# haidog-yaqub/EzAudio

Hardware: AMD Instinct MI355X
Metric: denoising steps/sec (EzAudio-XL, 10 s latent, CFG on) (higher is better)
Workload: dtype bf16

## Files before the change

ezaudio_amd/csrc/attn.hip:

```cpp
#include "common.h"

namespace {

typedef __attribute__((ext_vector_type(4))) short s16x4;

__device__ __forceinline__ float pair_max(float x) {
    const auto r = __builtin_amdgcn_permlane32_swap(__float_as_uint(x), __float_as_uint(x), false, false);
    return fmaxf(__uint_as_float(r[0]), __uint_as_float(r[1]));
}
__device__ __forceinline__ float pair_sum(float x) {
    const auto r = __builtin_amdgcn_permlane32_swap(__float_as_uint(x), __float_as_uint(x), false, false);
    return __uint_as_float(r[0]) + __uint_as_float(r[1]);
}

template <int DH>
struct HeadGeom;
template <>
struct HeadGeom<64> { static constexpr int DQK = 64, DV = 64; };
template <>
struct HeadGeom<72> { static constexpr int DQK = 80, DV = 96; };

template <int DH, int NKH, bool ZQ = false, int QT = 64>
__global__ __launch_bounds__(128 * NKH) void k_attn(AttnArgs a) {
    static_assert(QT == 64 || (QT == 32 && NKH == 4), "32-query tiles: the 8-wave fused-projection form only");
    constexpr int NQS = QT / 32;
    constexpr int NT = 128 * NKH;
    constexpr int TK = 32 * NKH;
    constexpr int DQK = HeadGeom<DH>::DQK;
    constexpr int DV = HeadGeom<DH>::DV;
    constexpr int NKS = DQK / 16;
    constexpr int NDT = DV / 32;
    constexpr int KSTR = DQK * 2 + 16;
    constexpr int VSTR = 192;
    static_assert(DV * 2 <= VSTR, "V row");
    constexpr int KBYTES = TK * KSTR, VBYTES = TK * VSTR;
    constexpr int BUF = KBYTES + VBYTES;
    constexpr int KCH = TK * DQK * 2 / 16;
    constexpr int VCPR = DV / 8;
    constexpr int VCH = TK * VCPR;
    constexpr int KPT = (KCH + NT - 1) / NT, VPT = (VCH + NT - 1) / NT;
    static_assert(KPT <= 3 && VPT <= 3, "staging registers");
    constexpr int DN = DV >= 96 ? 96 : 64;
    constexpr int DW = DQK;
    constexpr int DS = DQK;
    constexpr int NRS = QT == 64 ? 3 : 4;
    constexpr int PSTAGE = (QT + DN) * 128, PRING = 2 * NRS * PSTAGE;
    constexpr int PRED = 4 * 64 * DS * 4, PQS = QT * DQK * 2;
    constexpr int SMEM = NKH == 4 ? (2 * BUF > PRED + PQS ? (2 * BUF > PRING ? 2 * BUF : PRING) : (PRED + PQS > PRING ? PRED + PQS : PRING)) : 2 * BUF;
    constexpr int ZX = ZQ ? QT * 8 + 2 * DQK * 4 : 0;
    __shared__ __attribute__((aligned(16))) char smem[SMEM + ZX];

    int Lq_ = a.Lq;
    asm("" : "+s"(Lq_) : "s"(a.q), "s"(a.k), "s"(a.v), "s"(a.kmask), "s"(a.out), "s"(a.ldo), "s"(a.B), "s"(a.H), "s"(a.Lk), "s"(a.Lqp), "s"(a.Lkp), "s"(a.xu), "s"(a.ldu),
        "s"(a.xw), "s"(a.ldw), "s"(a.xw_rows), "s"(a.xK), "s"(a.xcd_map), "s"(a.nq), "s"(a.ppx), "s"(a.mnq), "s"(a.mH), "s"(a.q_raw), "s"(a.ts), "s"(a.xk2), "s"(a.zstat_in),
        "s"(a.zs_stride), "s"(a.zparts), "s"(a.klen));
    const int tid = threadIdx.x;
    const int lane = tid & 63;
    const int wave = tid >> 6;
    const int qs = QT == 64 ? (wave & 1) : 0, kh = QT == 64 ? (wave >> 1) : (wave & 3);
    const bool active = QT == 64 || __builtin_amdgcn_readfirstlane(wave) < 4;
    const int r32 = lane & 31, hi = lane >> 5;
    int qt, h, b;
    if (a.xcd_map) {
        const int xcd = blockIdx.x & 7, sl = blockIdx.x >> 3;
        const int sq = ez_div(sl, a.mnq);
        const int pair = xcd * a.ppx + sq;
        qt = sl - sq * a.nq;
        if (pair >= a.B * a.H) return;
        b = ez_div(pair, a.mH); h = pair - b * a.H;
    } else {
        qt = blockIdx.x; h = blockIdx.y; b = blockIdx.z;
    }
    const int q0 = qt * QT + qs * 32;
    const long bh = (long)b * a.H + h;
    int Lk = a.Lk;
    if constexpr (!ZQ) {
        if (a.klen) {
            Lk = __builtin_amdgcn_readfirstlane(a.klen[b]);
            if (qt * QT >= Lk) {
                for (int i = tid; i < QT * (DH / 4); i += NT) {
                    const int r = i / (DH / 4), g = i - r * (DH / 4);
                    if (qt * QT + r < a.Lq)
                        *reinterpret_cast<uint2*>(a.out + ((long)b * a.Lq + qt * QT + r) * a.ldo + h * DH + 4 * g) = make_uint2(0u, 0u);
                }
                return;
            }
        }
    }
    unsigned long long* ts = (a.ts && tid < 64) ? a.ts + 8 * (long)blockIdx.x : nullptr;
    if (ts && lane == 0) { ts[0] = __builtin_readcyclecounter(); ts[6] = ez_stamp_start(); }

    const bf16_t* Q = a.q + (bh * a.Lqp + q0 + r32) * DQK + 8 * hi;
    const char* Kg = reinterpret_cast<const char*>(a.k + bh * a.Lkp * DQK);
    const bf16_t* Vg = a.v + bh * DV * (long)a.Lkp;
    const uint8_t* km = a.kmask ? a.kmask + (long)b * a.Lk : nullptr;

    bf16x8 qf[NKS];
    if (NKH == 4 && a.xu) {
        if constexpr (NKH == 4) {
            constexpr int FN = DN / 32;
            constexpr int NPART = QT == 64 ? 4 : 8;
            const int rowb = b * a.Lq;
            float2* zrow_l = reinterpret_cast<float2*>(smem + SMEM);
            float* zgc_l = reinterpret_cast<float*>(smem + SMEM + QT * 8);
            ZStatRegs zst;
            float4 zgc_reg = make_float4(0.f, 0.f, 0.f, 0.f);
            const int wave_u = __builtin_amdgcn_readfirstlane(wave);
            const char* gA = reinterpret_cast<const char*>(a.xu);
            const char* gW = reinterpret_cast<const char*>(a.xw);
            const int nt = a.xK / 64;
            auto z_request = [&]() {
                if constexpr (ZQ) {
                    if (tid < 4 * QT) {
                        int qr = qt * QT + (tid >> 2);
                        qr = qr < a.Lq ? qr : a.Lq - 1;
                        z_row_stats_load(a.zstat_in + (rowb + qr), a.zs_stride, a.zparts, tid & 3, zst);
                    }
                    if (tid < 2 * (DH / 4)) {
                        const int which = tid >= DH / 4, t4 = tid - which * (DH / 4);
                        zgc_reg = *reinterpret_cast<const float4*>((which ? a.zC : a.zG) + h * DH + 4 * t4);
                    }
                }
            };
            f32x16 acc[FN];
#pragma unroll
            for (int j = 0; j < FN; ++j)
#pragma unroll
                for (int r = 0; r < 16; ++r) acc[j][r] = 0.f;
            if constexpr (QT == 32) {
                constexpr int NCH = (32 + DW) * 8, NW1 = (NCH - NT) / 64;
                static_assert(NCH > NT && NCH <= 2 * NT && (NCH - NT) % 64 == 0, "two passes, whole waves");
                uint32_t off0, off1;
                {
                    const int row = tid >> 3, c = tid & 7;
                    if (row < 32) {
                        int grow = rowb + qt * 32 + row;
                        grow = grow < rowb + a.Lq - 1 ? grow : rowb + a.Lq - 1;
                        off0 = (uint32_t)(grow * a.ldu + ((c ^ ((row >> 1) & 7)) << 3)) * 2u;
                    } else {
                        const int r2 = row - 32;
                        int gr = h * DH + r2;
                        gr = gr < a.xw_rows - 1 ? gr : a.xw_rows - 1;
                        off0 = (uint32_t)(gr * a.ldw + ((c ^ ((r2 >> 1) & 7)) << 3)) * 2u;
                    }
                    const int r2 = (tid >> 3) + 32;
                    int gr = h * DH + r2;
                    gr = gr < a.xw_rows - 1 ? gr : a.xw_rows - 1;
                    off1 = (uint32_t)(gr * a.ldw + ((c ^ ((r2 >> 1) & 7)) << 3)) * 2u;
                }
                const char* g0 = wave_u < 4 ? gA : gW;
                const bool two = wave_u < NW1;
                auto stage2 = [&](int sidx) {
                    char* dst = smem + (sidx % NRS) * 2 * PSTAGE + wave_u * 1024;
#pragma unroll
                    for (int sub = 0; sub < 2; ++sub) {
                        const long ko = (long)(2 * sidx + sub) * 128;
                        __builtin_amdgcn_global_load_lds((const __attribute__((address_space(1))) void*)(g0 + ko + off0),
                                                         (__attribute__((address_space(3))) void*)(dst + sub * PSTAGE), 16, 0, 0);
                        if (two)
                            __builtin_amdgcn_global_load_lds((const __attribute__((address_space(1))) void*)(gW + ko + off1),
                                                             (__attribute__((address_space(3))) void*)(dst + sub * PSTAGE + NT * 16), 16, 0, 0);
                    }
                };
                const int ns = nt >> 1;
                stage2(0);
                z_request();
                if (ns > 1) stage2(1);
                if (ns > 2) stage2(2);
                const int sub = wave_u >> 2, kq = wave_u & 3;
                const uint32_t fo = r32 * 128 + (((2 * kq + hi) ^ ((r32 >> 1) & 7)) << 4);
                for (int sidx = 0; sidx < ns; ++sidx) {
                    const int younger = ns - 1 - sidx < NRS - 2 ? ns - 1 - sidx : NRS - 2;
                    if (two) {
                        if (younger >= 2) asm volatile("s_waitcnt vmcnt(8)" ::: "memory");
                        else if (younger == 1) asm volatile("s_waitcnt vmcnt(4)" ::: "memory");
                        else asm volatile("s_waitcnt vmcnt(0)" ::: "memory");
                    } else {
                        if (younger >= 2) asm volatile("s_waitcnt vmcnt(4)" ::: "memory");
                        else if (younger == 1) asm volatile("s_waitcnt vmcnt(2)" ::: "memory");
                        else asm volatile("s_waitcnt vmcnt(0)" ::: "memory");
                    }
                    __builtin_amdgcn_s_barrier();
                    if (sidx + NRS - 1 < ns) stage2(sidx + NRS - 1);
                    const char* cT = smem + (sidx % NRS) * 2 * PSTAGE + sub * PSTAGE;
                    const bf16x8 af = *reinterpret_cast<const bf16x8*>(cT + fo);
#pragma unroll
                    for (int j = 0; j < FN; ++j) {
                        const bf16x8 bfr = *reinterpret_cast<const bf16x8*>(cT + 32 * 128 + fo + j * 4096);
                        acc[j] = __builtin_amdgcn_mfma_f32_32x32x16_bf16(bfr, af, acc[j], 0, 0, 0);
                    }
#pragma unroll
                    for (int j = 0; j < FN; ++j) asm volatile("" : "+a"(acc[j]));
                }
            } else {
            const int mh = wave & 1, kq = wave >> 1;
            uint32_t aoff[1], boff[(DW * 8 + NT - 1) / NT];
            stage_offsets<64, NT>(aoff, a.ldu, rowb + qt * 64, rowb + a.Lq - 1, tid);
            stage_offsets<DW, NT>(boff, a.ldw, h * DH, a.xw_rows - 1, tid);
            auto stage = [&](int t) {
                char* dst = smem + (t % 3) * PSTAGE + wave_u * 1024;
                stage_tile<64, NT>(gA + (long)t * 128, aoff, dst, tid);
                stage_tile<DW, NT>(gW + (long)t * 128, boff, dst + 64 * 128, tid);
            };
            const bool two = (DW * 8 > NT) && (wave_u * 64 + NT < DW * 8);
            stage(0);
            if (nt > 1) stage(1);
            z_request();
            const uint32_t fo = r32 * 128 + (((2 * kq + hi) ^ ((r32 >> 1) & 7)) << 4);
            if (a.xk2 && (nt & 1) == 0) {
                const int ns = nt >> 1;
                auto stage2 = [&](int sidx) {
                    char* dst = smem + (sidx % 3) * 2 * PSTAGE + wave_u * 1024;
#pragma unroll
                    for (int sub = 0; sub < 2; ++sub) {
                        stage_tile<64, NT>(gA + (long)(2 * sidx + sub) * 128, aoff, dst + sub * PSTAGE, tid);
                        stage_tile<DW, NT>(gW + (long)(2 * sidx + sub) * 128, boff, dst + sub * PSTAGE + 64 * 128, tid);
                    }
                };
                if (ns > 1) stage2(1);
                for (int sidx = 0; sidx < ns; ++sidx) {
                    if (sidx + 1 < ns) {
                        if (two) asm volatile("s_waitcnt vmcnt(6)" ::: "memory"); else asm volatile("s_waitcnt vmcnt(4)" ::: "memory");
                    } else {
                        asm volatile("s_waitcnt vmcnt(0)" ::: "memory");
                    }
                    __builtin_amdgcn_s_barrier();
                    if (sidx + 2 < ns) stage2(sidx + 2);
#pragma unroll
                    for (int sub = 0; sub < 2; ++sub) {
                        const char* cT = smem + (sidx % 3) * 2 * PSTAGE + sub * PSTAGE;
                        const bf16x8 af = *reinterpret_cast<const bf16x8*>(cT + fo + mh * 4096);
#pragma unroll
                        for (int j = 0; j < FN; ++j) {
                            const bf16x8 bfr = *reinterpret_cast<const bf16x8*>(cT + 64 * 128 + fo + j * 4096);
                            acc[j] = __builtin_amdgcn_mfma_f32_32x32x16_bf16(bfr, af, acc[j], 0, 0, 0);
                        }
                    }
#pragma unroll
                    for (int j = 0; j < FN; ++j) asm volatile("" : "+a"(acc[j]));
                }
            } else
            for (int t = 0; t < nt; ++t) {
                if (t + 1 < nt) {
                    if (two) asm volatile("s_waitcnt vmcnt(3)" ::: "memory"); else asm volatile("s_waitcnt vmcnt(2)" ::: "memory");
                } else {
                    asm volatile("s_waitcnt vmcnt(0)" ::: "memory");
                }
                __builtin_amdgcn_s_barrier();
                if (t + 2 < nt) stage(t + 2);
                const char* cT = smem + (t % 3) * PSTAGE;
                const bf16x8 af = *reinterpret_cast<const bf16x8*>(cT + fo + mh * 4096);
#pragma unroll
                for (int j = 0; j < FN; ++j) {
                    const bf16x8 bfr = *reinterpret_cast<const bf16x8*>(cT + 64 * 128 + fo + j * 4096);
                    acc[j] = __builtin_amdgcn_mfma_f32_32x32x16_bf16(bfr, af, acc[j], 0, 0, 0);
                }
#pragma unroll
                for (int j = 0; j < FN; ++j) asm volatile("" : "+a"(acc[j]));
            }
            }
#pragma unroll
            for (int j = 0; j < FN; ++j) asm volatile("s_nop 7\n\ts_nop 7\n\ts_nop 3" : "+a"(acc[j]));
            if constexpr (ZQ) {
                if (tid < 4 * QT) {
                    const float2 mr = z_row_stats_finish(zst, a.zparts, tid & 3, a.zD, a.zeps);
                    if ((tid & 3) == 0) zrow_l[tid >> 2] = mr;
                }
                if (tid < 2 * (DH / 4)) {
                    const int which = tid >= DH / 4, t4 = tid - which * (DH / 4);
                    *reinterpret_cast<float4*>(zgc_l + which * DQK + 4 * t4) = zgc_reg;
                }
            }
            __syncthreads();
            float* red = reinterpret_cast<float*>(smem);
            {
                const int pw = QT == 64 ? (wave >> 1) : wave, prow = QT == 64 ? 32 * (wave & 1) + r32 : r32;
#pragma unroll
                for (int j = 0; j < FN; ++j)
#pragma unroll
                    for (int g = 0; g < 4; ++g) {
                        const int col = 32 * j + 8 * g + 4 * hi;
                        if (col < DS)
                            *reinterpret_cast<float4*>(red + ((pw * QT + prow) * DS + col)) =
                                make_float4(acc[j][4 * g], acc[j][4 * g + 1], acc[j][4 * g + 2], acc[j][4 * g + 3]);
                    }
            }
            __syncthreads();
            if (QT == 64 || tid < 8 * QT) {
                constexpr int CP = DH / 8;
                bf16_t* qs_l = reinterpret_cast<bf16_t*>(smem + PRED);
                const int row = tid >> 3, part = tid & 7;
                float v[CP];
                float s1 = 0.f;
                const float2 zmr = ZQ ? zrow_l[row] : make_float2(0.f, 1.f);
                const float zmu = zmr.x, zr = zmr.y;
#pragma unroll
                for (int e = 0; e < CP; ++e) {
                    const int col = part * CP + e;
                    if constexpr (QT == 64) {
                        v[e] = red[(0 * 64 + row) * DS + col] + red[(1 * 64 + row) * DS + col] + red[(2 * 64 + row) * DS + col] +
                               red[(3 * 64 + row) * DS + col];
                    } else {
                        float t = red[row * DS + col];
#pragma unroll
                        for (int w = 1; w < NPART; ++w) t += red[(w * QT + row) * DS + col];
                        v[e] = t;
                    }
                    if constexpr (ZQ) v[e] = fmaf(zr, v[e], fmaf(-zr * zmu, zgc_l[col], zgc_l[DQK + col]));
                    s1 += v[e];
                }
                s1 = oct_sum(s1);
                const float mean = s1 * (1.f / DH);
                float s2 = 0.f;
#pragma unroll
                for (int e = 0; e < CP; ++e) { const float d = v[e] - mean; s2 += d * d; }
                s2 = oct_sum(s2);
                const float rstd = rsqrtf(s2 * (1.f / DH) + 1e-5f);
#pragma unroll
                for (int e = 0; e < CP; ++e) {
                    const int col = part * CP + e;
                    qs_l[row * DQK + col] = f2bf((v[e] - mean) * rstd * a.qn_w[col] + a.qn_b[col]);
                }
                if (DQK > DH && part == 0)
                    for (int col = DH; col < DQK; ++col) qs_l[row * DQK + col] = 0;
            }
            __syncthreads();
            {
                const bf16_t* qs_l = reinterpret_cast<const bf16_t*>(smem + PRED);
#pragma unroll
                for (int ks = 0; ks < NKS; ++ks) qf[ks] = *reinterpret_cast<const bf16x8*>(qs_l + (32 * qs + r32) * DQK + 16 * ks + 8 * hi);
            }
            __syncthreads();
        }
    } else if (a.q_raw) {
        int qr = q0 + r32;
        if (qr >= a.Lq) qr = a.Lq - 1;
        const float* src = a.q_raw + ((long)b * a.Lq + qr) * a.ld_qraw + h * DH + 8 * hi;
        float v[NKS][8];
        float s = 0.f;
#pragma unroll
        for (int ks = 0; ks < NKS; ++ks) {
            const bool ok = 16 * ks + 8 * hi < DH;
            const float4 lo = ok ? *reinterpret_cast<const float4*>(src + 16 * ks) : make_float4(0.f, 0.f, 0.f, 0.f);
            const float4 hh = ok ? *reinterpret_cast<const float4*>(src + 16 * ks + 4) : make_float4(0.f, 0.f, 0.f, 0.f);
            v[ks][0] = lo.x; v[ks][1] = lo.y; v[ks][2] = lo.z; v[ks][3] = lo.w;
            v[ks][4] = hh.x; v[ks][5] = hh.y; v[ks][6] = hh.z; v[ks][7] = hh.w;
#pragma unroll
            for (int e = 0; e < 8; ++e) s += v[ks][e];
        }
        s += __shfl_xor(s, 32, 64);
        const float mean = s * (1.f / DH);
        float q2 = 0.f;
#pragma unroll
        for (int ks = 0; ks < NKS; ++ks)
            if (16 * ks + 8 * hi < DH) {
#pragma unroll
                for (int e = 0; e < 8; ++e) { const float d = v[ks][e] - mean; q2 += d * d; }
            }
        q2 += __shfl_xor(q2, 32, 64);
        const float rstd = rsqrtf(q2 * (1.f / DH) + 1e-5f);
#pragma unroll
        for (int ks = 0; ks < NKS; ++ks) {
            const int d0 = 16 * ks + 8 * hi;
            const bool ok = d0 < DH;
            const int dw = ok ? d0 : 0;
            union { bf16x8 v; uint32_t u[4]; } pk;
#pragma unroll
            for (int e = 0; e < 4; ++e) {
                const float y0 = ok ? (v[ks][2 * e] - mean) * rstd * a.qn_w[dw + 2 * e] + a.qn_b[dw + 2 * e] : 0.f;
                const float y1 = ok ? (v[ks][2 * e + 1] - mean) * rstd * a.qn_w[dw + 2 * e + 1] + a.qn_b[dw + 2 * e + 1] : 0.f;
                pk.u[e] = pack_bf2(y0, y1);
            }
            qf[ks] = pk.v;
        }
    } else {
#pragma unroll
        for (int ks = 0; ks < NKS; ++ks) qf[ks] = *reinterpret_cast<const bf16x8*>(Q + 16 * ks);
    }

    uint4 k0 = {}, k1 = {}, k2 = {}, v0 = {}, v1 = {}, v2 = {};
    uint32_t koff[3], voff[3];
#pragma unroll
    for (int i = 0; i < 3; ++i) {
        int ck = tid + NT * i, cv = tid + NT * i;
        ck = ck < KCH ? ck : KCH - 1;
        cv = cv < VCH ? cv : VCH - 1;
        koff[i] = (uint32_t)ck * 16u;
        voff[i] = (uint32_t)cv * 16u;
    }
    const __amdgpu_buffer_rsrc_t krs = __builtin_amdgcn_make_buffer_rsrc(const_cast<char*>(Kg), 0, a.Lkp * DQK * 2, 0x00020000);
    const __amdgpu_buffer_rsrc_t vrs = __builtin_amdgcn_make_buffer_rsrc(const_cast<bf16_t*>(Vg), 0, DV * a.Lkp * 2, 0x00020000);
    auto kchunk = [&](int i, int key0) -> uint4 {
        return __builtin_bit_cast(uint4, __builtin_amdgcn_raw_buffer_load_b128(krs, (int)koff[i], key0 * DQK * 2, 0));
    };
    auto vchunk = [&](int i, int key0) -> uint4 {
        return __builtin_bit_cast(uint4, __builtin_amdgcn_raw_buffer_load_b128(vrs, (int)voff[i], key0 * DV * 2, 0));
    };
    auto kstore = [&](int i, char* kb, const uint4& val) {
        const int c = tid + NT * i;
        if (c < KCH) *reinterpret_cast<uint4*>(kb + (c / (DQK / 8)) * KSTR + (c % (DQK / 8)) * 16) = val;
    };
    auto vstore = [&](int i, char* vb, const uint4& val) {
        const int c = tid + NT * i;
        if (c < VCH) *reinterpret_cast<uint4*>(vb + (c / VCPR) * VSTR + (c % VCPR) * 16) = val;
    };
#define LOAD_TILE(t)                                   \
    do {                                               \
        const int key0_ = (t) * TK;                    \
        k0 = kchunk(0, key0_);                         \
        k1 = kchunk(1, key0_);                         \
        if constexpr (KPT > 2) k2 = kchunk(2, key0_);  \
        v0 = vchunk(0, key0_);                         \
        v1 = vchunk(1, key0_);                         \
        if constexpr (VPT > 2) v2 = vchunk(2, key0_);  \
    } while (0)
#define WRITE_TILE(buf)                                \
    do {                                               \
        char* kb_ = smem + (buf) * BUF;                \
        char* vb_ = kb_ + KBYTES;                      \
        kstore(0, kb_, k0);                            \
        kstore(1, kb_, k1);                            \
        if constexpr (KPT > 2) kstore(2, kb_, k2);     \
        vstore(0, vb_, v0);                            \
        vstore(1, vb_, v1);                            \
        if constexpr (VPT > 2) vstore(2, vb_, v2);     \
    } while (0)

    f32x16 o[NDT];
#pragma unroll
    for (int t = 0; t < NDT; ++t)
#pragma unroll
        for (int r = 0; r < 16; ++r) o[t][r] = 0.f;
    float m = -1e30f, lsum = 0.f;
    constexpr float RESCALE_THR = 4.0f;
    const float c = 1.4426950408889634f * rsqrtf((float)DH);

    if (NKH == 4 && __builtin_amdgcn_readfirstlane(threadIdx.x) >= 256) __builtin_amdgcn_s_setprio(1);
    const int ntiles = (Lk + TK - 1) / TK;
    LOAD_TILE(0);
    WRITE_TILE(0);
    __syncthreads();
    if (ts && lane == 0) ts[1] = __builtin_readcyclecounter();
    for (int t = 0; t < ntiles; ++t) {
        if (t + 1 < ntiles) LOAD_TILE(t + 1);
        const char* kb = smem + (t & 1) * BUF;
        const char* vb = kb + KBYTES;
        const char* vtr = vb + (32 * kh + 4 * hi + ((lane & 15) >> 2)) * VSTR + ((lane & 16) + 4 * (lane & 3)) * 2;
        const int key0 = t * TK + kh * 32;
        if (active && key0 < Lk) {
            const int kidx = key0 + r32;
            bool kv = kidx < Lk;
            if (km) kv = kv && (km[kidx < Lk ? kidx : 0] != 0);
            const uint32_t ball = (uint32_t)__ballot(kv);
            const uint32_t tmask = ball >> (4 * hi);
            const bool full = ball == 0xffffffffu;
            f32x16 s;
            {
                const bf16x8 kf0 = *reinterpret_cast<const bf16x8*>(kb + (kh * 32 + r32) * KSTR + hi * 16);
                asm("s_nop 1\n\tv_mfma_f32_32x32x16_bf16 %0, %1, %2, 0" : "=&v"(s) : "v"(kf0), "v"(qf[0]));
            }
#pragma unroll
            for (int ks = 1; ks < NKS; ++ks) {
                const bf16x8 kf = *reinterpret_cast<const bf16x8*>(kb + (kh * 32 + r32) * KSTR + (2 * ks + hi) * 16);
                if (ks + 1 < NKS) asm("s_nop 1\n\tv_mfma_f32_32x32x16_bf16 %0, %1, %2, %0" : "+v"(s) : "v"(kf), "v"(qf[ks]));
                else asm("s_nop 1\n\tv_mfma_f32_32x32x16_bf16 %0, %1, %2, %0\n\ts_nop 7\n\ts_nop 7\n\ts_nop 3" : "+v"(s) : "v"(kf), "v"(qf[ks]));
            }
            float tmax = -1e30f;
            if (full) {
#pragma unroll
                for (int r = 0; r < 16; ++r) tmax = fmaxf(tmax, s[r]);
                tmax *= c;
            } else {
#pragma unroll
                for (int r = 0; r < 16; ++r) {
                    const bool v = (tmask >> ((r & 3) + 8 * (r >> 2))) & 1u;
                    s[r] = v ? s[r] * c : -1e30f;
                    tmax = fmaxf(tmax, s[r]);
                }
            }
            tmax = pair_max(tmax);
            if (!__all(tmax <= m + RESCALE_THR)) {
                const float mnew = fmaxf(m, tmax);
                const float alpha = __builtin_amdgcn_exp2f(m - mnew);
                m = mnew;
                lsum *= alpha;
#pragma unroll
                for (int tt = 0; tt < NDT; ++tt)
#pragma unroll
                    for (int r = 0; r < 16; ++r) o[tt][r] *= alpha;
            }
            float psum = 0.f;
            float p[16];
            if (full) {
                const f32x2 c2 = {c, c}, nm2 = {-m, -m};
                f32x2 ps2 = {0.f, 0.f};
#pragma unroll
                for (int r = 0; r < 16; r += 2) {
                    f32x2 x = {s[r], s[r + 1]};
                    x = __builtin_elementwise_fma(x, c2, nm2);
                    p[r] = __builtin_amdgcn_exp2f(x[0]);
                    p[r + 1] = __builtin_amdgcn_exp2f(x[1]);
                    const f32x2 pp = {p[r], p[r + 1]};
                    ps2 += pp;
                }
                psum = ps2[0] + ps2[1];
// ... 78 lines not shown
                }
                if (a.wt) st8_wt(orow + 8 * G, v); else *reinterpret_cast<uint2*>(orow + 8 * G) = v;
            }
        }
    }
    if (ts && lane == 0) { asm volatile("s_waitcnt vmcnt(0)" ::: "memory"); ts[3] = __builtin_readcyclecounter(); ts[7] = __builtin_amdgcn_s_memrealtime(); }
}

#undef LOAD_TILE
#undef WRITE_TILE

}

int launch_attention(const AttnArgs& a0, hipStream_t st) {
    AttnArgs a = a0;
    if (a.b0 > 0) {
        const int DQK = a.dh == 64 ? 64 : 80, DV = a.dh == 64 ? 64 : 96;
        const long b0 = a.b0;
        if (a.q) a.q += b0 * a.H * a.Lqp * DQK;
        if (a.k) a.k += b0 * a.H * a.Lkp * DQK;
        if (a.v) a.v += b0 * a.H * DV * (long)a.Lkp;
        if (a.kmask) a.kmask += b0 * a.Lk;
        if (a.out) a.out += b0 * a.Lq * a.ldo;
        if (a.q_raw) a.q_raw += b0 * a.Lq * a.ld_qraw;
        if (a.xu) a.xu += b0 * a.Lq * a.ldu;
        if (a.zstat_in) a.zstat_in += b0 * a.Lq;
        if (a.klen) a.klen += b0;
        a.b0 = 0;
    }
    const long nwg64 = (long)((a.Lq + 63) / 64) * a.H * a.B;
    int nkh = a.nkh;
    if (nkh != 2 && nkh != 4) nkh = nwg64 <= 512 ? 4 : 2;
    if (a.Lkp % 128) nkh = 2;
    if (a.xu && nkh != 4) return 1;
    if (a.dh != 64 && a.dh != 72) return 1;
    if (a.klen && (a.xu || a.q_raw || a.Lq != a.Lk)) return 1;
    const bool zq = a.xu && a.zstat_in;
    if (zq && !(a.zG && a.zC && a.zparts > 0 && a.zparts <= Z_MAXP && a.zs_stride > 0 && a.zw > 0)) return 1;
    const bool q32 = zq && nkh == 4 && (a.xK / 64) % 2 == 0 && a.xcd_map && (a.qtile == 32 || (a.qtile == 0 && nwg64 <= 128));
    const int QT = q32 ? 32 : 64;
    a.nq = (a.Lq + QT - 1) / QT;
    a.ppx = (a.B * a.H + 7) / 8;
    a.mnq = ez_magic(a.nq); a.mH = ez_magic(a.H);
    dim3 grid(a.nq, a.H, a.B);
    if (a.xcd_map) grid = dim3(8 * a.ppx * a.nq, 1, 1);
    if (a.ts && (long)grid.x * grid.y * grid.z > a.ts_cap) a.ts = nullptr;
    if (q32) {
        if (a.dh == 64) hipLaunchKernelGGL((k_attn<64, 4, true, 32>), grid, dim3(512), 0, st, a);
        else hipLaunchKernelGGL((k_attn<72, 4, true, 32>), grid, dim3(512), 0, st, a);
        return 0;
    }
    if (a.dh == 64) {
        if (nkh == 4 && zq) hipLaunchKernelGGL((k_attn<64, 4, true>), grid, dim3(512), 0, st, a);
        else if (nkh == 4) hipLaunchKernelGGL((k_attn<64, 4>), grid, dim3(512), 0, st, a);
        else hipLaunchKernelGGL((k_attn<64, 2>), grid, dim3(256), 0, st, a);
    } else {
        if (nkh == 4 && zq) hipLaunchKernelGGL((k_attn<72, 4, true>), grid, dim3(512), 0, st, a);
        else if (nkh == 4) hipLaunchKernelGGL((k_attn<72, 4>), grid, dim3(512), 0, st, a);
        else hipLaunchKernelGGL((k_attn<72, 2>), grid, dim3(256), 0, st, a);
    }
    return 0;
}
```

Measured before the change: 269.4.

## Overlap first K/V tile and mask loads with fused Q projection prologue

```diff
diff --git a/ezaudio_amd/csrc/attn.hip b/ezaudio_amd/csrc/attn.hip
--- a/ezaudio_amd/csrc/attn.hip
+++ b/ezaudio_amd/csrc/attn.hip
@@ -20,8 +20,9 @@
 template <>
 struct HeadGeom<72> { static constexpr int DQK = 80, DV = 96; };
 
-template <int DH, int NKH, bool ZQ = false, int QT = 64>
+template <int DH, int NKH, bool ZQ = false, int QT = 64, bool XU = ZQ>
 __global__ __launch_bounds__(128 * NKH) void k_attn(AttnArgs a) {
+    static_assert((!ZQ || XU) && (!XU || NKH == 4), "the fused projection: 8-wave form; the LayerNorm algebra: fused projection only");
     static_assert(QT == 64 || (QT == 32 && NKH == 4), "32-query tiles: the 8-wave fused-projection form only");
     constexpr int NQS = QT / 32;
     constexpr int NT = 128 * NKH;
@@ -47,13 +48,17 @@
     constexpr int PSTAGE = (QT + DN) * 128, PRING = 2 * NRS * PSTAGE;
     constexpr int PRED = 4 * 64 * DS * 4, PQS = QT * DQK * 2;
     constexpr int SMEM = NKH == 4 ? (2 * BUF > PRED + PQS ? (2 * BUF > PRING ? 2 * BUF : PRING) : (PRED + PQS > PRING ? PRED + PQS : PRING)) : 2 * BUF;
-    constexpr int ZX = ZQ ? QT * 8 + 2 * DQK * 4 : 0;
+    constexpr int ZXZ = ZQ ? QT * 8 + 2 * DQK * 4 : 0;
+    constexpr int ZX = ZXZ + (XU ? 2 * DQK * 4 : 0);
     __shared__ __attribute__((aligned(16))) char smem[SMEM + ZX];
 
     int Lq_ = a.Lq;
     asm("" : "+s"(Lq_) : "s"(a.q), "s"(a.k), "s"(a.v), "s"(a.kmask), "s"(a.out), "s"(a.ldo), "s"(a.B), "s"(a.H), "s"(a.Lk), "s"(a.Lqp), "s"(a.Lkp), "s"(a.xu), "s"(a.ldu),
         "s"(a.xw), "s"(a.ldw), "s"(a.xw_rows), "s"(a.xK), "s"(a.xcd_map), "s"(a.nq), "s"(a.ppx), "s"(a.mnq), "s"(a.mH), "s"(a.q_raw), "s"(a.ts), "s"(a.xk2), "s"(a.zstat_in),
         "s"(a.zs_stride), "s"(a.zparts), "s"(a.klen));
+    const float* qn_w_ = a.qn_w;
+    const float* qn_b_ = a.qn_b;
+    asm("" : "+s"(qn_w_), "+s"(qn_b_));
     const int tid = threadIdx.x;
     const int lane = tid & 63;
     const int wave = tid >> 6;
@@ -94,289 +99,6 @@
     const char* Kg = reinterpret_cast<const char*>(a.k + bh * a.Lkp * DQK);
     const bf16_t* Vg = a.v + bh * DV * (long)a.Lkp;
     const uint8_t* km = a.kmask ? a.kmask + (long)b * a.Lk : nullptr;
-
-    bf16x8 qf[NKS];
-    if (NKH == 4 && a.xu) {
-        if constexpr (NKH == 4) {
-            constexpr int FN = DN / 32;
-            constexpr int NPART = QT == 64 ? 4 : 8;
-            const int rowb = b * a.Lq;
-            float2* zrow_l = reinterpret_cast<float2*>(smem + SMEM);
-            float* zgc_l = reinterpret_cast<float*>(smem + SMEM + QT * 8);
-            ZStatRegs zst;
-            float4 zgc_reg = make_float4(0.f, 0.f, 0.f, 0.f);
-            const int wave_u = __builtin_amdgcn_readfirstlane(wave);
-            const char* gA = reinterpret_cast<const char*>(a.xu);
-            const char* gW = reinterpret_cast<const char*>(a.xw);
-            const int nt = a.xK / 64;
-            auto z_request = [&]() {
-                if constexpr (ZQ) {
-                    if (tid < 4 * QT) {
-                        int qr = qt * QT + (tid >> 2);
-                        qr = qr < a.Lq ? qr : a.Lq - 1;
-                        z_row_stats_load(a.zstat_in + (rowb + qr), a.zs_stride, a.zparts, tid & 3, zst);
-                    }
-                    if (tid < 2 * (DH / 4)) {
-                        const int which = tid >= DH / 4, t4 = tid - which * (DH / 4);
-                        zgc_reg = *reinterpret_cast<const float4*>((which ? a.zC : a.zG) + h * DH + 4 * t4);
-                    }
-                }
-            };
-            f32x16 acc[FN];
-#pragma unroll
-            for (int j = 0; j < FN; ++j)
-#pragma unroll
-                for (int r = 0; r < 16; ++r) acc[j][r] = 0.f;
-            if constexpr (QT == 32) {
-                constexpr int NCH = (32 + DW) * 8, NW1 = (NCH - NT) / 64;
-                static_assert(NCH > NT && NCH <= 2 * NT && (NCH - NT) % 64 == 0, "two passes, whole waves");
-                uint32_t off0, off1;
-                {
-                    const int row = tid >> 3, c = tid & 7;
-                    if (row < 32) {
-                        int grow = rowb + qt * 32 + row;
-                        grow = grow < rowb + a.Lq - 1 ? grow : rowb + a.Lq - 1;
-                        off0 = (uint32_t)(grow * a.ldu + ((c ^ ((row >> 1) & 7)) << 3)) * 2u;
-                    } else {
-                        const int r2 = row - 32;
-                        int gr = h * DH + r2;
-                        gr = gr < a.xw_rows - 1 ? gr : a.xw_rows - 1;
-                        off0 = (uint32_t)(gr * a.ldw + ((c ^ ((r2 >> 1) & 7)) << 3)) * 2u;
-                    }
-                    const int r2 = (tid >> 3) + 32;
-                    int gr = h * DH + r2;
-                    gr = gr < a.xw_rows - 1 ? gr : a.xw_rows - 1;
-                    off1 = (uint32_t)(gr * a.ldw + ((c ^ ((r2 >> 1) & 7)) << 3)) * 2u;
-                }
-                const char* g0 = wave_u < 4 ? gA : gW;
-                const bool two = wave_u < NW1;
-                auto stage2 = [&](int sidx) {
-                    char* dst = smem + (sidx % NRS) * 2 * PSTAGE + wave_u * 1024;
-#pragma unroll
-                    for (int sub = 0; sub < 2; ++sub) {
-                        const long ko = (long)(2 * sidx + sub) * 128;
-                        __builtin_amdgcn_global_load_lds((const __attribute__((address_space(1))) void*)(g0 + ko + off0),
-                                                         (__attribute__((address_space(3))) void*)(dst + sub * PSTAGE), 16, 0, 0);
-                        if (two)
-                            __builtin_amdgcn_global_load_lds((const __attribute__((address_space(1))) void*)(gW + ko + off1),
-                                                             (__attribute__((address_space(3))) void*)(dst + sub * PSTAGE + NT * 16), 16, 0, 0);
-                    }
-                };
-                const int ns = nt >> 1;
-                stage2(0);
-                z_request();
-                if (ns > 1) stage2(1);
-                if (ns > 2) stage2(2);
-                const int sub = wave_u >> 2, kq = wave_u & 3;
-                const uint32_t fo = r32 * 128 + (((2 * kq + hi) ^ ((r32 >> 1) & 7)) << 4);
-                for (int sidx = 0; sidx < ns; ++sidx) {
-                    const int younger = ns - 1 - sidx < NRS - 2 ? ns - 1 - sidx : NRS - 2;
-                    if (two) {
-                        if (younger >= 2) asm volatile("s_waitcnt vmcnt(8)" ::: "memory");
-                        else if (younger == 1) asm volatile("s_waitcnt vmcnt(4)" ::: "memory");
-                        else asm volatile("s_waitcnt vmcnt(0)" ::: "memory");
-                    } else {
-                        if (younger >= 2) asm volatile("s_waitcnt vmcnt(4)" ::: "memory");
-                        else if (younger == 1) asm volatile("s_waitcnt vmcnt(2)" ::: "memory");
-                        else asm volatile("s_waitcnt vmcnt(0)" ::: "memory");
-                    }
-                    __builtin_amdgcn_s_barrier();
-                    if (sidx + NRS - 1 < ns) stage2(sidx + NRS - 1);
-                    const char* cT = smem + (sidx % NRS) * 2 * PSTAGE + sub * PSTAGE;
-                    const bf16x8 af = *reinterpret_cast<const bf16x8*>(cT + fo);
-#pragma unroll
-                    for (int j = 0; j < FN; ++j) {
-                        const bf16x8 bfr = *reinterpret_cast<const bf16x8*>(cT + 32 * 128 + fo + j * 4096);
-                        acc[j] = __builtin_amdgcn_mfma_f32_32x32x16_bf16(bfr, af, acc[j], 0, 0, 0);
-                    }
-#pragma unroll
-                    for (int j = 0; j < FN; ++j) asm volatile("" : "+a"(acc[j]));
-                }
-            } else {
-            const int mh = wave & 1, kq = wave >> 1;
-            uint32_t aoff[1], boff[(DW * 8 + NT - 1) / NT];
-            stage_offsets<64, NT>(aoff, a.ldu, rowb + qt * 64, rowb + a.Lq - 1, tid);
-            stage_offsets<DW, NT>(boff, a.ldw, h * DH, a.xw_rows - 1, tid);
-            auto stage = [&](int t) {
-                char* dst = smem + (t % 3) * PSTAGE + wave_u * 1024;
-                stage_tile<64, NT>(gA + (long)t * 128, aoff, dst, tid);
-                stage_tile<DW, NT>(gW + (long)t * 128, boff, dst + 64 * 128, tid);
-            };
-            const bool two = (DW * 8 > NT) && (wave_u * 64 + NT < DW * 8);
-            stage(0);
-            if (nt > 1) stage(1);
-            z_request();
-            const uint32_t fo = r32 * 128 + (((2 * kq + hi) ^ ((r32 >> 1) & 7)) << 4);
-            if (a.xk2 && (nt & 1) == 0) {
-                const int ns = nt >> 1;
-                auto stage2 = [&](int sidx) {
-                    char* dst = smem + (sidx % 3) * 2 * PSTAGE + wave_u * 1024;
-#pragma unroll
-                    for (int sub = 0; sub < 2; ++sub) {
-                        stage_tile<64, NT>(gA + (long)(2 * sidx + sub) * 128, aoff, dst + sub * PSTAGE, tid);
-                        stage_tile<DW, NT>(gW + (long)(2 * sidx + sub) * 128, boff, dst + sub * PSTAGE + 64 * 128, tid);
-                    }
-                };
-                if (ns > 1) stage2(1);
-                for (int sidx = 0; sidx < ns; ++sidx) {
-                    if (sidx + 1 < ns) {
-                        if (two) asm volatile("s_waitcnt vmcnt(6)" ::: "memory"); else asm volatile("s_waitcnt vmcnt(4)" ::: "memory");
-                    } else {
-                        asm volatile("s_waitcnt vmcnt(0)" ::: "memory");
-                    }
-                    __builtin_amdgcn_s_barrier();
-                    if (sidx + 2 < ns) stage2(sidx + 2);
-#pragma unroll
-                    for (int sub = 0; sub < 2; ++sub) {
-                        const char* cT = smem + (sidx % 3) * 2 * PSTAGE + sub * PSTAGE;
-                        const bf16x8 af = *reinterpret_cast<const bf16x8*>(cT + fo + mh * 4096);
-#pragma unroll
-                        for (int j = 0; j < FN; ++j) {
-                            const bf16x8 bfr = *reinterpret_cast<const bf16x8*>(cT + 64 * 128 + fo + j * 4096);
-                            acc[j] = __builtin_amdgcn_mfma_f32_32x32x16_bf16(bfr, af, acc[j], 0, 0, 0);
-                        }
-                    }
-#pragma unroll
-                    for (int j = 0; j < FN; ++j) asm volatile("" : "+a"(acc[j]));
-                }
-            } else
-            for (int t = 0; t < nt; ++t) {
-                if (t + 1 < nt) {
-                    if (two) asm volatile("s_waitcnt vmcnt(3)" ::: "memory"); else asm volatile("s_waitcnt vmcnt(2)" ::: "memory");
-                } else {
-                    asm volatile("s_waitcnt vmcnt(0)" ::: "memory");
-                }
-                __builtin_amdgcn_s_barrier();
-                if (t + 2 < nt) stage(t + 2);
-                const char* cT = smem + (t % 3) * PSTAGE;
-                const bf16x8 af = *reinterpret_cast<const bf16x8*>(cT + fo + mh * 4096);
-#pragma unroll
-                for (int j = 0; j < FN; ++j) {
-                    const bf16x8 bfr = *reinterpret_cast<const bf16x8*>(cT + 64 * 128 + fo + j * 4096);
-                    acc[j] = __builtin_amdgcn_mfma_f32_32x32x16_bf16(bfr, af, acc[j], 0, 0, 0);
-                }
-#pragma unroll
-                for (int j = 0; j < FN; ++j) asm volatile("" : "+a"(acc[j]));
-            }
-            }
-#pragma unroll
-            for (int j = 0; j < FN; ++j) asm volatile("s_nop 7\n\ts_nop 7\n\ts_nop 3" : "+a"(acc[j]));
-            if constexpr (ZQ) {
-                if (tid < 4 * QT) {
-                    const float2 mr = z_row_stats_finish(zst, a.zparts, tid & 3, a.zD, a.zeps);
-                    if ((tid & 3) == 0) zrow_l[tid >> 2] = mr;
-                }
-                if (tid < 2 * (DH / 4)) {
-                    const int which = tid >= DH / 4, t4 = tid - which * (DH / 4);
-                    *reinterpret_cast<float4*>(zgc_l + which * DQK + 4 * t4) = zgc_reg;
-                }
-            }
-            __syncthreads();
-            float* red = reinterpret_cast<float*>(smem);
-            {
-                const int pw = QT == 64 ? (wave >> 1) : wave, prow = QT == 64 ? 32 * (wave & 1) + r32 : r32;
-#pragma unroll
-                for (int j = 0; j < FN; ++j)
-#pragma unroll
-                    for (int g = 0; g < 4; ++g) {
-                        const int col = 32 * j + 8 * g + 4 * hi;
-                        if (col < DS)
-                            *reinterpret_cast<float4*>(red + ((pw * QT + prow) * DS + col)) =
-                                make_float4(acc[j][4 * g], acc[j][4 * g + 1], acc[j][4 * g + 2], acc[j][4 * g + 3]);
-                    }
-            }
-            __syncthreads();
-            if (QT == 64 || tid < 8 * QT) {
-                constexpr int CP = DH / 8;
-                bf16_t* qs_l = reinterpret_cast<bf16_t*>(smem + PRED);
-                const int row = tid >> 3, part = tid & 7;
-                float v[CP];
-                float s1 = 0.f;
-                const float2 zmr = ZQ ? zrow_l[row] : make_float2(0.f, 1.f);
-                const float zmu = zmr.x, zr = zmr.y;
-#pragma unroll
-                for (int e = 0; e < CP; ++e) {
-                    const int col = part * CP + e;
-                    if constexpr (QT == 64) {
-                        v[e] = red[(0 * 64 + row) * DS + col] + red[(1 * 64 + row) * DS + col] + red[(2 * 64 + row) * DS + col] +
-                               red[(3 * 64 + row) * DS + col];
-                    } else {
-                        float t = red[row * DS + col];
-#pragma unroll
-                        for (int w = 1; w < NPART; ++w) t += red[(w * QT + row) * DS + col];
-                        v[e] = t;
-                    }
-                    if constexpr (ZQ) v[e] = fmaf(zr, v[e], fmaf(-zr * zmu, zgc_l[col], zgc_l[DQK + col]));
-                    s1 += v[e];
-                }
-                s1 = oct_sum(s1);
-                const float mean = s1 * (1.f / DH);
-                float s2 = 0.f;
-#pragma unroll
-                for (int e = 0; e < CP; ++e) { const float d = v[e] - mean; s2 += d * d; }
-                s2 = oct_sum(s2);
-                const float rstd = rsqrtf(s2 * (1.f / DH) + 1e-5f);
-#pragma unroll
-                for (int e = 0; e < CP; ++e) {
-                    const int col = part * CP + e;
-                    qs_l[row * DQK + col] = f2bf((v[e] - mean) * rstd * a.qn_w[col] + a.qn_b[col]);
-                }
-                if (DQK > DH && part == 0)
-                    for (int col = DH; col < DQK; ++col) qs_l[row * DQK + col] = 0;
-            }
-            __syncthreads();
-            {
-                const bf16_t* qs_l = reinterpret_cast<const bf16_t*>(smem + PRED);
-#pragma unroll
-                for (int ks = 0; ks < NKS; ++ks) qf[ks] = *reinterpret_cast<const bf16x8*>(qs_l + (32 * qs + r32) * DQK + 16 * ks + 8 * hi);
-            }
-            __syncthreads();
-        }
-    } else if (a.q_raw) {
-        int qr = q0 + r32;
-        if (qr >= a.Lq) qr = a.Lq - 1;
-        const float* src = a.q_raw + ((long)b * a.Lq + qr) * a.ld_qraw + h * DH + 8 * hi;
-        float v[NKS][8];
-        float s = 0.f;
-#pragma unroll
-        for (int ks = 0; ks < NKS; ++ks) {
-            const bool ok = 16 * ks + 8 * hi < DH;
-            const float4 lo = ok ? *reinterpret_cast<const float4*>(src + 16 * ks) : make_float4(0.f, 0.f, 0.f, 0.f);
-            const float4 hh = ok ? *reinterpret_cast<const float4*>(src + 16 * ks + 4) : make_float4(0.f, 0.f, 0.f, 0.f);
-            v[ks][0] = lo.x; v[ks][1] = lo.y; v[ks][2] = lo.z; v[ks][3] = lo.w;
-            v[ks][4] = hh.x; v[ks][5] = hh.y; v[ks][6] = hh.z; v[ks][7] = hh.w;
-#pragma unroll
-            for (int e = 0; e < 8; ++e) s += v[ks][e];
-        }
-        s += __shfl_xor(s, 32, 64);
-        const float mean = s * (1.f / DH);
-        float q2 = 0.f;
-#pragma unroll
-        for (int ks = 0; ks < NKS; ++ks)
-            if (16 * ks + 8 * hi < DH) {
-#pragma unroll
-                for (int e = 0; e < 8; ++e) { const float d = v[ks][e] - mean; q2 += d * d; }
-            }
-        q2 += __shfl_xor(q2, 32, 64);
-        const float rstd = rsqrtf(q2 * (1.f / DH) + 1e-5f);
-#pragma unroll
-        for (int ks = 0; ks < NKS; ++ks) {
-            const int d0 = 16 * ks + 8 * hi;
-            const bool ok = d0 < DH;
-            const int dw = ok ? d0 : 0;
-            union { bf16x8 v; uint32_t u[4]; } pk;
-#pragma unroll
-            for (int e = 0; e < 4; ++e) {
-                const float y0 = ok ? (v[ks][2 * e] - mean) * rstd * a.qn_w[dw + 2 * e] + a.qn_b[dw + 2 * e] : 0.f;
-                const float y1 = ok ? (v[ks][2 * e + 1] - mean) * rstd * a.qn_w[dw + 2 * e + 1] + a.qn_b[dw + 2 * e + 1] : 0.f;
-                pk.u[e] = pack_bf2(y0, y1);
-            }
-            qf[ks] = pk.v;
-        }
-    } else {
-#pragma unroll
-        for (int ks = 0; ks < NKS; ++ks) qf[ks] = *reinterpret_cast<const bf16x8*>(Q + 16 * ks);
-    }
 
     uint4 k0 = {}, k1 = {}, k2 = {}, v0 = {}, v1 = {}, v2 = {};
     uint32_t koff[3], voff[3];
@@ -425,6 +147,336 @@
         vstore(1, vb_, v1);                            \
         if constexpr (VPT > 2) vstore(2, vb_, v2);     \
     } while (0)
+    uint32_t mk0 = 0;
+
+    bf16x8 qf[NKS];
+    if constexpr (XU) {
+        {
+            constexpr int FN = DN / 32;
+            constexpr int NPART = QT == 64 ? 4 : 8;
+            const int rowb = b * a.Lq;
+            float2* zrow_l = reinterpret_cast<float2*>(smem + SMEM);
+            float* zgc_l = reinterpret_cast<float*>(smem + SMEM + QT * 8);
+            static_assert(Z_PT == 3, "three blind statistics loads per thread");
+            f32x2 ez0, ez1, ez2;
+            f32x4 ezgc;
+            const int wave_u = __builtin_amdgcn_readfirstlane(wave);
+            const char* gA = reinterpret_cast<const char*>(a.xu);
+            const char* gW = reinterpret_cast<const char*>(a.xw);
+            const int nt = a.xK / 64;
+            auto z_request = [&]() {
+                if constexpr (ZQ) {
+                    {
+                        int qr = qt * QT + (tid >> 2);
+                        qr = qr < a.Lq ? qr : a.Lq - 1;
+                        const float2* st = a.zstat_in + (rowb + qr);
+                        const int pg = tid & 3, pl = a.zparts - 1;
+                        asm volatile("global_load_dwordx2 %0, %1, off" : "=a"(ez0) : "v"(st + (pg < pl ? pg : pl) * a.zs_stride) : "memory");
+                        asm volatile("global_load_dwordx2 %0, %1, off" : "=a"(ez1) : "v"(st + (pg + 4 < pl ? pg + 4 : pl) * a.zs_stride) : "memory");
+                        asm volatile("global_load_dwordx2 %0, %1, off" : "=a"(ez2) : "v"(st + (pg + 8 < pl ? pg + 8 : pl) * a.zs_stride) : "memory");
+                    }
+                    {
+                        const int tq = tid < 2 * (DH / 4) ? tid : 2 * (DH / 4) - 1;
+                        const int which = tq >= DH / 4, t4 = tq - which * (DH / 4);
+                        asm volatile("global_load_dwordx4 %0, %1, off" : "=a"(ezgc) : "v"((which ? a.zC : a.zG) + h * DH + 4 * t4) : "memory");
+                    }
+                }
+            };
+            f32x4 ek0, ek1, ek2, ev0, ev1, ev2, eqn;
+            uint32_t emk;
+            float* qn_l = reinterpret_cast<float*>(smem + SMEM + ZXZ);
+            auto early_request = [&]() {
+                asm volatile("s_nop 4\n\tbuffer_load_dwordx4 %0, %1, %2, 0 offen" : "=a"(ek0) : "v"(koff[0]), "s"(krs) : "memory");
+                asm volatile("buffer_load_dwordx4 %0, %1, %2, 0 offen" : "=a"(ek1) : "v"(koff[1]), "s"(krs) : "memory");
+                if constexpr (KPT > 2) asm volatile("buffer_load_dwordx4 %0, %1, %2, 0 offen" : "=a"(ek2) : "v"(koff[2]), "s"(krs) : "memory");
+                asm volatile("s_nop 4\n\tbuffer_load_dwordx4 %0, %1, %2, 0 offen" : "=a"(ev0) : "v"(voff[0]), "s"(vrs) : "memory");
+                asm volatile("buffer_load_dwordx4 %0, %1, %2, 0 offen" : "=a"(ev1) : "v"(voff[1]), "s"(vrs) : "memory");
+                if constexpr (VPT > 2) asm volatile("buffer_load_dwordx4 %0, %1, %2, 0 offen" : "=a"(ev2) : "v"(voff[2]), "s"(vrs) : "memory");
+                {
+                    const int kidx = kh * 32 + r32;
+                    const uint8_t* mp = km ? km + (kidx < Lk ? kidx : 0) : reinterpret_cast<const uint8_t*>(Kg);
+                    asm volatile("global_load_ubyte %0, %1, off" : "=a"(emk) : "v"(mp) : "memory");
+                }
+                {
+                    const int tq = tid < 2 * (DH / 4) ? tid : 2 * (DH / 4) - 1;
+                    const int which = tq >= DH / 4, t4 = tq - which * (DH / 4);
+                    asm volatile("global_load_dwordx4 %0, %1, off" : "=a"(eqn) : "v"((which ? qn_b_ : qn_w_) + 4 * t4) : "memory");
+                }
+            };
+            f32x16 acc[FN];
+#pragma unroll
+            for (int j = 0; j < FN; ++j)
+#pragma unroll
+                for (int r = 0; r < 16; ++r) acc[j][r] = 0.f;
+            if constexpr (QT == 32) {
+                constexpr int NCH = (32 + DW) * 8, NW1 = (NCH - NT) / 64;
+                static_assert(NCH > NT && NCH <= 2 * NT && (NCH - NT) % 64 == 0, "two passes, whole waves");
+                uint32_t off0, off1;
+                {
+                    const int row = tid >> 3, c = tid & 7;
+                    if (row < 32) {
+                        int grow = rowb + qt * 32 + row;
+                        grow = grow < rowb + a.Lq - 1 ? grow : rowb + a.Lq - 1;
+                        off0 = (uint32_t)(grow * a.ldu + ((c ^ ((row >> 1) & 7)) << 3)) * 2u;
+                    } else {
+                        const int r2 = row - 32;
+                        int gr = h * DH + r2;
+                        gr = gr < a.xw_rows - 1 ? gr : a.xw_rows - 1;
+                        off0 = (uint32_t)(gr * a.ldw + ((c ^ ((r2 >> 1) & 7)) << 3)) * 2u;
+                    }
+                    const int r2 = (tid >> 3) + 32;
+                    int gr = h * DH + r2;
+                    gr = gr < a.xw_rows - 1 ? gr : a.xw_rows - 1;
+                    off1 = (uint32_t)(gr * a.ldw + ((c ^ ((r2 >> 1) & 7)) << 3)) * 2u;
+                }
+                const char* g0 = wave_u < 4 ? gA : gW;
+                const bool two = wave_u < NW1;
+                auto stage2 = [&](int sidx) {
+                    char* dst = smem + (sidx % NRS) * 2 * PSTAGE + wave_u * 1024;
+#pragma unroll
+                    for (int sub = 0; sub < 2; ++sub) {
+                        const long ko = (long)(2 * sidx + sub) * 128;
+                        __builtin_amdgcn_global_load_lds((const __attribute__((address_space(1))) void*)(g0 + ko + off0),
+                                                         (__attribute__((address_space(3))) void*)(dst + sub * PSTAGE), 16, 0, 0);
+                        if (two)
+                            __builtin_amdgcn_global_load_lds((const __attribute__((address_space(1))) void*)(gW + ko + off1),
+                                                             (__attribute__((address_space(3))) void*)(dst + sub * PSTAGE + NT * 16), 16, 0, 0);
+                    }
+                };
+                const int ns = nt >> 1;
+                stage2(0);
+                z_request();
+                early_request();
+                if (ns > 1) stage2(1);
+                if (ns > 2) stage2(2);
+                const int sub = wave_u >> 2, kq = wave_u & 3;
+                const uint32_t fo = r32 * 128 + (((2 * kq + hi) ^ ((r32 >> 1) & 7)) << 4);
+                for (int sidx = 0; sidx < ns; ++sidx) {
+                    const int younger = ns - 1 - sidx < NRS - 2 ? ns - 1 - sidx : NRS - 2;
+                    if (two) {
+                        if (younger >= 2) asm volatile("s_waitcnt vmcnt(8)" ::: "memory");
+                        else if (younger == 1) asm volatile("s_waitcnt vmcnt(4)" ::: "memory");
+                        else asm volatile("s_waitcnt vmcnt(0)" ::: "memory");
+                    } else {
+                        if (younger >= 2) asm volatile("s_waitcnt vmcnt(4)" ::: "memory");
+                        else if (younger == 1) asm volatile("s_waitcnt vmcnt(2)" ::: "memory");
+                        else asm volatile("s_waitcnt vmcnt(0)" ::: "memory");
+                    }
+                    __builtin_amdgcn_s_barrier();
+                    if (sidx + NRS - 1 < ns) stage2(sidx + NRS - 1);
+                    const char* cT = smem + (sidx % NRS) * 2 * PSTAGE + sub * PSTAGE;
+                    const bf16x8 af = *reinterpret_cast<const bf16x8*>(cT + fo);
+#pragma unroll
+                    for (int j = 0; j < FN; ++j) {
+                        const bf16x8 bfr = *reinterpret_cast<const bf16x8*>(cT + 32 * 128 + fo + j * 4096);
+                        acc[j] = __builtin_amdgcn_mfma_f32_32x32x16_bf16(bfr, af, acc[j], 0, 0, 0);
+                    }
+#pragma unroll
+                    for (int j = 0; j < FN; ++j) asm volatile("" : "+a"(acc[j]));
+                }
+            } else {
+            const int mh = wave & 1, kq = wave >> 1;
+            uint32_t aoff[1], boff[(DW * 8 + NT - 1) / NT];
+            stage_offsets<64, NT>(aoff, a.ldu, rowb + qt * 64, rowb + a.Lq - 1, tid);
+            stage_offsets<DW, NT>(boff, a.ldw, h * DH, a.xw_rows - 1, tid);
+            auto stage = [&](int t) {
+                char* dst = smem + (t % 3) * PSTAGE + wave_u * 1024;
+                stage_tile<64, NT>(gA + (long)t * 128, aoff, dst, tid);
+                stage_tile<DW, NT>(gW + (long)t * 128, boff, dst + 64 * 128, tid);
+            };
+            const bool two = (DW * 8 > NT) && (wave_u * 64 + NT < DW * 8);
+            stage(0);
+            if (nt > 1) stage(1);
+            z_request();
+            early_request();
+            const uint32_t fo = r32 * 128 + (((2 * kq + hi) ^ ((r32 >> 1) & 7)) << 4);
+            if (a.xk2 && (nt & 1) == 0) {
+                const int ns = nt >> 1;
+                auto stage2 = [&](int sidx) {
+                    char* dst = smem + (sidx % 3) * 2 * PSTAGE + wave_u * 1024;
+#pragma unroll
+                    for (int sub = 0; sub < 2; ++sub) {
+                        stage_tile<64, NT>(gA + (long)(2 * sidx + sub) * 128, aoff, dst + sub * PSTAGE, tid);
+                        stage_tile<DW, NT>(gW + (long)(2 * sidx + sub) * 128, boff, dst + sub * PSTAGE + 64 * 128, tid);
+                    }
+                };
+                if (ns > 1) stage2(1);
+                for (int sidx = 0; sidx < ns; ++sidx) {
+                    if (sidx + 1 < ns) {
+                        if (two) asm volatile("s_waitcnt vmcnt(6)" ::: "memory"); else asm volatile("s_waitcnt vmcnt(4)" ::: "memory");
+                    } else {
+                        asm volatile("s_waitcnt vmcnt(0)" ::: "memory");
+                    }
+                    __builtin_amdgcn_s_barrier();
+                    if (sidx + 2 < ns) stage2(sidx + 2);
+#pragma unroll
+                    for (int sub = 0; sub < 2; ++sub) {
+                        const char* cT = smem + (sidx % 3) * 2 * PSTAGE + sub * PSTAGE;
+                        const bf16x8 af = *reinterpret_cast<const bf16x8*>(cT + fo + mh * 4096);
+#pragma unroll
+                        for (int j = 0; j < FN; ++j) {
+                            const bf16x8 bfr = *reinterpret_cast<const bf16x8*>(cT + 64 * 128 + fo + j * 4096);
+                            acc[j] = __builtin_amdgcn_mfma_f32_32x32x16_bf16(bfr, af, acc[j], 0, 0, 0);
+                        }
+                    }
+#pragma unroll
+                    for (int j = 0; j < FN; ++j) asm volatile("" : "+a"(acc[j]));
+                }
+            } else
+            for (int t = 0; t < nt; ++t) {
+                if (t + 1 < nt) {
+                    if (two) asm volatile("s_waitcnt vmcnt(3)" ::: "memory"); else asm volatile("s_waitcnt vmcnt(2)" ::: "memory");
+                } else {
+                    asm volatile("s_waitcnt vmcnt(0)" ::: "memory");
+                }
+                __builtin_amdgcn_s_barrier();
+                if (t + 2 < nt) stage(t + 2);
+                const char* cT = smem + (t % 3) * PSTAGE;
+                const bf16x8 af = *reinterpret_cast<const bf16x8*>(cT + fo + mh * 4096);
+#pragma unroll
+                for (int j = 0; j < FN; ++j) {
+                    const bf16x8 bfr = *reinterpret_cast<const bf16x8*>(cT + 64 * 128 + fo + j * 4096);
+                    acc[j] = __builtin_amdgcn_mfma_f32_32x32x16_bf16(bfr, af, acc[j], 0, 0, 0);
+                }
+#pragma unroll
+                for (int j = 0; j < FN; ++j) asm volatile("" : "+a"(acc[j]));
+            }
+            }
+#pragma unroll
+            for (int j = 0; j < FN; ++j) asm volatile("s_nop 7\n\ts_nop 7\n\ts_nop 3" : "+a"(acc[j]));
+            if constexpr (ZQ) {
+                asm volatile("s_waitcnt vmcnt(0)" : "+a"(ez0), "+a"(ez1), "+a"(ez2), "+a"(ezgc));
+                if (tid < 4 * QT) {
+                    ZStatRegs zst;
+                    zst.v[0] = make_float2(ez0[0], ez0[1]); zst.v[1] = make_float2(ez1[0], ez1[1]); zst.v[2] = make_float2(ez2[0], ez2[1]);
+                    const float2 mr = z_row_stats_finish(zst, a.zparts, tid & 3, a.zD, a.zeps);
+                    if ((tid & 3) == 0) zrow_l[tid >> 2] = mr;
+                }
+                if (tid < 2 * (DH / 4)) {
+                    const int which = tid >= DH / 4, t4 = tid - which * (DH / 4);
+                    *reinterpret_cast<f32x4*>(zgc_l + which * DQK + 4 * t4) = ezgc;
+                }
+            }
+            asm volatile("s_waitcnt vmcnt(0)" : "+a"(eqn));
+            if (tid < 2 * (DH / 4)) {
+                const int which = tid >= DH / 4, t4 = tid - which * (DH / 4);
+                *reinterpret_cast<f32x4*>(qn_l + which * DQK + 4 * t4) = eqn;
+            }
+            __syncthreads();
+            float* red = reinterpret_cast<float*>(smem);
+            {
+                const int pw = QT == 64 ? (wave >> 1) : wave, prow = QT == 64 ? 32 * (wave & 1) + r32 : r32;
+#pragma unroll
+                for (int j = 0; j < FN; ++j)
+#pragma unroll
+                    for (int g = 0; g < 4; ++g) {
+                        const int col = 32 * j + 8 * g + 4 * hi;
+                        if (col < DS)
+                            *reinterpret_cast<float4*>(red + ((pw * QT + prow) * DS + col)) =
+                                make_float4(acc[j][4 * g], acc[j][4 * g + 1], acc[j][4 * g + 2], acc[j][4 * g + 3]);
+                    }
+            }
+            __syncthreads();
+            if (QT == 64 || tid < 8 * QT) {
+                constexpr int CP = DH / 8;
+                bf16_t* qs_l = reinterpret_cast<bf16_t*>(smem + PRED);
+                const int row = tid >> 3, part = tid & 7;
+                float v[CP];
+                float s1 = 0.f;
+                const float2 zmr = ZQ ? zrow_l[row] : make_float2(0.f, 1.f);
+                const float zmu = zmr.x, zr = zmr.y;
+#pragma unroll
+                for (int e = 0; e < CP; ++e) {
+                    const int col = part * CP + e;
+                    if constexpr (QT == 64) {
+                        v[e] = red[(0 * 64 + row) * DS + col] + red[(1 * 64 + row) * DS + col] + red[(2 * 64 + row) * DS + col] +
+                               red[(3 * 64 + row) * DS + col];
+                    } else {
+                        float t = red[row * DS + col];
+#pragma unroll
+                        for (int w = 1; w < NPART; ++w) t += red[(w * QT + row) * DS + col];
+                        v[e] = t;
+                    }
+                    if constexpr (ZQ) v[e] = fmaf(zr, v[e], fmaf(-zr * zmu, zgc_l[col], zgc_l[DQK + col]));
+                    s1 += v[e];
+                }
+                s1 = oct_sum(s1);
+                const float mean = s1 * (1.f / DH);
+                float s2 = 0.f;
+#pragma unroll
+                for (int e = 0; e < CP; ++e) { const float d = v[e] - mean; s2 += d * d; }
+                s2 = oct_sum(s2);
+                const float rstd = rsqrtf(s2 * (1.f / DH) + 1e-5f);
+#pragma unroll
+                for (int e = 0; e < CP; ++e) {
+                    const int col = part * CP + e;
+                    qs_l[row * DQK + col] = f2bf((v[e] - mean) * rstd * qn_l[col] + qn_l[DQK + col]);
+                }
+                if (DQK > DH && part == 0)
+                    for (int col = DH; col < DQK; ++col) qs_l[row * DQK + col] = 0;
+            }
+            __syncthreads();
+            {
+                const bf16_t* qs_l = reinterpret_cast<const bf16_t*>(smem + PRED);
+#pragma unroll
+                for (int ks = 0; ks < NKS; ++ks) qf[ks] = *reinterpret_cast<const bf16x8*>(qs_l + (32 * qs + r32) * DQK + 16 * ks + 8 * hi);
+            }
+            __syncthreads();
+            if constexpr (KPT > 2 && VPT > 2) asm volatile("s_waitcnt vmcnt(0)" : "+a"(ek0), "+a"(ek1), "+a"(ek2), "+a"(ev0), "+a"(ev1), "+a"(ev2), "+a"(emk));
+            else if constexpr (KPT > 2) asm volatile("s_waitcnt vmcnt(0)" : "+a"(ek0), "+a"(ek1), "+a"(ek2), "+a"(ev0), "+a"(ev1), "+a"(emk));
+            else if constexpr (VPT > 2) asm volatile("s_waitcnt vmcnt(0)" : "+a"(ek0), "+a"(ek1), "+a"(ev0), "+a"(ev1), "+a"(ev2), "+a"(emk));
+            else asm volatile("s_waitcnt vmcnt(0)" : "+a"(ek0), "+a"(ek1), "+a"(ev0), "+a"(ev1), "+a"(emk));
+            k0 = __builtin_bit_cast(uint4, ek0); k1 = __builtin_bit_cast(uint4, ek1);
+            if constexpr (KPT > 2) k2 = __builtin_bit_cast(uint4, ek2);
+            v0 = __builtin_bit_cast(uint4, ev0); v1 = __builtin_bit_cast(uint4, ev1);
+            if constexpr (VPT > 2) v2 = __builtin_bit_cast(uint4, ev2);
+            mk0 = emk;
+        }
+    } else if (a.q_raw) {
+        int qr = q0 + r32;
+        if (qr >= a.Lq) qr = a.Lq - 1;
+        const float* src = a.q_raw + ((long)b * a.Lq + qr) * a.ld_qraw + h * DH + 8 * hi;
+        float v[NKS][8];
+        float s = 0.f;
+#pragma unroll
+        for (int ks = 0; ks < NKS; ++ks) {
+            const bool ok = 16 * ks + 8 * hi < DH;
+            const float4 lo = ok ? *reinterpret_cast<const float4*>(src + 16 * ks) : make_float4(0.f, 0.f, 0.f, 0.f);
+            const float4 hh = ok ? *reinterpret_cast<const float4*>(src + 16 * ks + 4) : make_float4(0.f, 0.f, 0.f, 0.f);
+            v[ks][0] = lo.x; v[ks][1] = lo.y; v[ks][2] = lo.z; v[ks][3] = lo.w;
+            v[ks][4] = hh.x; v[ks][5] = hh.y; v[ks][6] = hh.z; v[ks][7] = hh.w;
+#pragma unroll
+            for (int e = 0; e < 8; ++e) s += v[ks][e];
+        }
+        s += __shfl_xor(s, 32, 64);
+        const float mean = s * (1.f / DH);
+        float q2 = 0.f;
+#pragma unroll
+        for (int ks = 0; ks < NKS; ++ks)
+            if (16 * ks + 8 * hi < DH) {
+#pragma unroll
+                for (int e = 0; e < 8; ++e) { const float d = v[ks][e] - mean; q2 += d * d; }
+            }
+        q2 += __shfl_xor(q2, 32, 64);
+        const float rstd = rsqrtf(q2 * (1.f / DH) + 1e-5f);
+#pragma unroll
+        for (int ks = 0; ks < NKS; ++ks) {
+            const int d0 = 16 * ks + 8 * hi;
+            const bool ok = d0 < DH;
+            const int dw = ok ? d0 : 0;
+            union { bf16x8 v; uint32_t u[4]; } pk;
+#pragma unroll
+            for (int e = 0; e < 4; ++e) {
+                const float y0 = ok ? (v[ks][2 * e] - mean) * rstd * a.qn_w[dw + 2 * e] + a.qn_b[dw + 2 * e] : 0.f;
+                const float y1 = ok ? (v[ks][2 * e + 1] - mean) * rstd * a.qn_w[dw + 2 * e + 1] + a.qn_b[dw + 2 * e + 1] : 0.f;
+                pk.u[e] = pack_bf2(y0, y1);
+            }
+            qf[ks] = pk.v;
+        }
+    } else {
+#pragma unroll
+        for (int ks = 0; ks < NKS; ++ks) qf[ks] = *reinterpret_cast<const bf16x8*>(Q + 16 * ks);
+    }
 
     f32x16 o[NDT];
 #pragma unroll
@@ -437,7 +489,7 @@
 
     if (NKH == 4 && __builtin_amdgcn_readfirstlane(threadIdx.x) >= 256) __builtin_amdgcn_s_setprio(1);
     const int ntiles = (Lk + TK - 1) / TK;
-    LOAD_TILE(0);
+    if constexpr (!XU) LOAD_TILE(0);
     WRITE_TILE(0);
     __syncthreads();
     if (ts && lane == 0) ts[1] = __builtin_readcyclecounter();
@@ -450,7 +502,11 @@
         if (active && key0 < Lk) {
             const int kidx = key0 + r32;
             bool kv = kidx < Lk;
-            if (km) kv = kv && (km[kidx < Lk ? kidx : 0] != 0);
+            if (km) {
+                uint32_t mb;
+                if (XU && t == 0) mb = mk0; else mb = km[kidx < Lk ? kidx : 0];
+                kv = kv && (mb != 0);
+            }
             const uint32_t ball = (uint32_t)__ballot(kv);
             const uint32_t tmask = ball >> (4 * hi);
             const bool full = ball == 0xffffffffu;
@@ -635,10 +691,12 @@
     }
     if (a.dh == 64) {
         if (nkh == 4 && zq) hipLaunchKernelGGL((k_attn<64, 4, true>), grid, dim3(512), 0, st, a);
+        else if (nkh == 4 && a.xu) hipLaunchKernelGGL((k_attn<64, 4, false, 64, true>), grid, dim3(512), 0, st, a);
         else if (nkh == 4) hipLaunchKernelGGL((k_attn<64, 4>), grid, dim3(512), 0, st, a);
         else hipLaunchKernelGGL((k_attn<64, 2>), grid, dim3(256), 0, st, a);
     } else {
         if (nkh == 4 && zq) hipLaunchKernelGGL((k_attn<72, 4, true>), grid, dim3(512), 0, st, a);
+        else if (nkh == 4 && a.xu) hipLaunchKernelGGL((k_attn<72, 4, false, 64, true>), grid, dim3(512), 0, st, a);
         else if (nkh == 4) hipLaunchKernelGGL((k_attn<72, 4>), grid, dim3(512), 0, st, a);
         else hipLaunchKernelGGL((k_attn<72, 2>), grid, dim3(256), 0, st, a);
     }
```

New measurement: 271.0, median of 6. About the same (+0.6%).
